# YuHang-max/3DSAD-main

Hardware: AMD Instinct MI355X
Metric: scenes/sec (16384-pt KITTI-shaped) through SA+cluster path (higher is better)
Workload: dtype f32

## Files before the change

3dsad-main_amd/csrc/ball_query.hip:

```cpp
#include "common.h"

namespace {

struct BQParams {
    float radii[SAD_MAX_RADII];
    int nsample[SAD_MAX_RADII];
    int32_t *idx[SAD_MAX_RADII];
    int32_t *cnt[SAD_MAX_RADII];
};

constexpr int BQ_WAVES = 4;

template <int NR, int CW>
__global__ __launch_bounds__(BQ_WAVES * 64) void ball_query_kernel(
    const float *__restrict__ xyz, const float *__restrict__ new_xyz,
    const float *__restrict__ radius_pc, BQParams prm, int N, int M) {
    const int lane = threadIdx.x & 63;
    const int wave = __builtin_amdgcn_readfirstlane(threadIdx.x >> 6);
    const int b = blockIdx.y;
    const int m0 = (blockIdx.x * BQ_WAVES + wave) * CW;
    const float *p = xyz + (size_t)b * N * 3;

    float cx[CW], cy[CW], cz[CW], r2[CW][NR];
    int cnt[CW][NR], first[CW][NR];
    bool active[CW];
    int ndone = 0;
#pragma unroll
    for (int c = 0; c < CW; ++c) {
        active[c] = (m0 + c) < M;
        const int m = active[c] ? m0 + c : M - 1;
        const float *q = new_xyz + ((size_t)b * M + m) * 3;
        cx[c] = q[0];
        cy[c] = q[1];
        cz[c] = q[2];
#pragma unroll
        for (int r = 0; r < NR; ++r) {
            float rad = prm.radii[r];
            if (radius_pc) rad = rad * radius_pc[(size_t)b * M + m];
            r2[c][r] = rad * rad;
            first[c][r] = 0;
            cnt[c][r] = active[c] ? 0 : prm.nsample[r];
            if (!active[c]) ++ndone;
        }
    }

    for (int base = 0; base < N && ndone < CW * NR; base += 64) {
        const int j = base + lane;
        const bool valid = j < N;
        const int jj = valid ? j : N - 1;
        const float px = p[jj * 3 + 0], py = p[jj * 3 + 1], pz = p[jj * 3 + 2];
#pragma unroll
        for (int c = 0; c < CW; ++c) {
            const float d = sad::d2f(px, py, pz, cx[c], cy[c], cz[c]);
#pragma unroll
            for (int r = 0; r < NR; ++r) {
                const bool in = valid && (d < r2[c][r]);
                const unsigned long long mask = __ballot(in);
                if (mask != 0ull && cnt[c][r] < prm.nsample[r]) {
                    const int slot = cnt[c][r] + __builtin_amdgcn_mbcnt_hi((unsigned)(mask >> 32), __builtin_amdgcn_mbcnt_lo((unsigned)mask, 0u));
                    if (in && slot < prm.nsample[r])
                        prm.idx[r][((size_t)b * M + (m0 + c)) * prm.nsample[r] + slot] = j;
                    if (cnt[c][r] == 0) first[c][r] = base + __builtin_ctzll(mask);
                    cnt[c][r] += __builtin_popcountll(mask);
                    if (cnt[c][r] >= prm.nsample[r]) ++ndone;
                }
            }
        }
    }
#pragma unroll
    for (int c = 0; c < CW; ++c) {
        if (!active[c]) continue;
#pragma unroll
        for (int r = 0; r < NR; ++r) {
            const int S = prm.nsample[r];
            const int n = cnt[c][r] < S ? cnt[c][r] : S;
            for (int s = n + lane; s < S; s += 64)
                prm.idx[r][((size_t)b * M + (m0 + c)) * S + s] = first[c][r];
            if (prm.cnt[r] && lane == 0) prm.cnt[r][(size_t)b * M + (m0 + c)] = n;
        }
    }
}

template <int NR>
void launch_bq(const float *xyz, const float *new_xyz, const float *radius_pc, const BQParams &prm,
               int B, int N, int M, hipStream_t st) {
    constexpr int CW = 4;
    dim3 grid((M + BQ_WAVES * CW - 1) / (BQ_WAVES * CW), B);
    hipLaunchKernelGGL((ball_query_kernel<NR, CW>), grid, dim3(BQ_WAVES * 64), 0, st, xyz, new_xyz,
                       radius_pc, prm, N, M);
}

__global__ __launch_bounds__(256) void knn_kernel(const float *__restrict__ xyz,
                                                  const float *__restrict__ new_xyz, int N, int M,
                                                  int K, int32_t *__restrict__ idx) {
    const int lane = threadIdx.x & 63;
    const int wave = __builtin_amdgcn_readfirstlane(threadIdx.x >> 6);
    const int b = blockIdx.y;
    const int m = blockIdx.x * 4 + wave;
    if (m >= M) return;
    const float *p = xyz + (size_t)b * N * 3;
    const float *q = new_xyz + ((size_t)b * M + m) * 3;
    const float cx = q[0], cy = q[1], cz = q[2];
    float ld = __builtin_inff();
    int lj = 0;
    float worst = __builtin_inff();
    int filled = 0;
    for (int base = 0; base < N; base += 64) {
        const int j = base + lane;
        const bool valid = j < N;
        const int jj = valid ? j : N - 1;
        const float d = sad::d2f(p[jj * 3 + 0], p[jj * 3 + 1], p[jj * 3 + 2], cx, cy, cz);
        unsigned long long mask = __ballot(valid && (d < worst || filled < K));
        while (mask) {
            const int l = __builtin_ctzll(mask);
            mask &= mask - 1;
            const float xd = __builtin_bit_cast(float, __builtin_amdgcn_readlane(__builtin_bit_cast(int, d), l));
            if (!(xd < worst) && filled >= K) continue;
            const int pos = __builtin_popcountll(__ballot(lane < filled && ld <= xd));
            const float ud = __shfl_up(ld, 1, 64);
            const int uj = __shfl_up(lj, 1, 64);
            if (lane > pos) {
                ld = ud;
                lj = uj;
            } else if (lane == pos) {
                ld = xd;
                lj = base + l;
            }
            if (lane >= K) ld = __builtin_inff();
            filled = filled < K ? filled + 1 : K;
            worst = filled < K ? __builtin_inff() : __builtin_bit_cast(float, __builtin_amdgcn_readlane(__builtin_bit_cast(int, ld), K - 1));
        }
    }
    if (lane < K) idx[((size_t)b * M + m) * K + lane] = lj;
}

int check_common(const char *fn, const void *xyz, const void *new_xyz, int B, int N, int M) {
    if (!xyz || !new_xyz) return sad::fail(SAD_EINVAL, "%s: NULL pointer", fn);
    if (B < 1 || N < 1 || M < 1) return sad::fail(SAD_EINVAL, "%s: need B,N,M >= 1 (B=%d N=%d M=%d)", fn, B, N, M);
    if (B > 65535) return sad::fail(SAD_EUNSUPPORTED, "%s: B=%d > 65535", fn, B);
    if ((size_t)N * 3 >= (1u << 31)) return sad::fail(SAD_EUNSUPPORTED, "%s: N too large", fn);
    return SAD_OK;
}

}

SAD_API int sad_ball_query_multi_f32(const float *xyz, const float *new_xyz, int n_radii,
                                     const float *radii, const float *radius_pc,
                                     const int *nsamples, int32_t *const *idx, int32_t *const *cnt,
                                     int B, int N, int M, sad_stream_t stream) {
    if (int e = check_common("sad_ball_query_multi_f32", xyz, new_xyz, B, N, M)) return e;
    SAD_REQUIRE(n_radii >= 1 && n_radii <= SAD_MAX_RADII, "sad_ball_query_multi_f32: n_radii=%d not in 1..%d", n_radii, SAD_MAX_RADII);
    SAD_REQUIRE(radii && nsamples && idx, "sad_ball_query_multi_f32: NULL parameter array");
    BQParams prm{};
    for (int r = 0; r < n_radii; ++r) {
        SAD_REQUIRE(nsamples[r] >= 1 && nsamples[r] <= 64, "sad_ball_query: nsample=%d not in 1..64", nsamples[r]);
        SAD_REQUIRE(idx[r], "sad_ball_query: NULL idx output");
        prm.radii[r] = radii[r];
        prm.nsample[r] = nsamples[r];
        prm.idx[r] = idx[r];
        prm.cnt[r] = cnt ? cnt[r] : nullptr;
    }
    hipStream_t st = (hipStream_t)stream;
    switch (n_radii) {
        case 1: launch_bq<1>(xyz, new_xyz, radius_pc, prm, B, N, M, st); break;
        case 2: launch_bq<2>(xyz, new_xyz, radius_pc, prm, B, N, M, st); break;
        case 3: launch_bq<3>(xyz, new_xyz, radius_pc, prm, B, N, M, st); break;
        default: launch_bq<4>(xyz, new_xyz, radius_pc, prm, B, N, M, st); break;
    }
    return sad::check_launch("sad_ball_query");
}

SAD_API int sad_ball_query_f32(const float *xyz, const float *new_xyz, float radius,
                               const float *radius_pc, int B, int N, int M, int S, int32_t *idx,
                               sad_stream_t stream) {
    const float radii[1] = {radius_pc ? 1.0f : radius};
    const int ns[1] = {S};
    int32_t *const outs[1] = {idx};
    return sad_ball_query_multi_f32(xyz, new_xyz, 1, radii, radius_pc, ns, outs, nullptr, B, N, M, stream);
}

SAD_API int sad_knn_f32(const float *xyz, const float *new_xyz, int B, int N, int M, int K,
                        int32_t *idx, sad_stream_t stream) {
    if (int e = check_common("sad_knn_f32", xyz, new_xyz, B, N, M)) return e;
    SAD_REQUIRE(idx, "sad_knn_f32: NULL idx");
    SAD_REQUIRE(K >= 1 && K <= 64 && K <= N, "sad_knn_f32: need 1 <= K <= min(64, N) (K=%d N=%d)", K, N);
    dim3 grid((M + 3) / 4, B);
    hipLaunchKernelGGL(knn_kernel, grid, dim3(256), 0, (hipStream_t)stream, xyz, new_xyz, N, M, K, idx);
    return sad::check_launch("sad_knn_f32");
}
```

Measured before the change: 8401.

## Stage small point clouds in registers and skip empty radius checks in ball query

For N up to 2048, each lane preloads all its point coordinates into registers up front, in NCH chunks, with an asm barrier to force the loads to issue early. The centroid width drops to 2 waves' worth on these paths. A per-centroid max-radius ballot lets a chunk skip all radius tests when no lane is inside, and also skips centroids whose radii are all full. Out-of-range lanes get NaN coordinates so the valid predicate can be dropped from the ballot. The aim is to cut global-load latency and redundant ballots, at the cost of higher register pressure and more template instantiations.

```diff
diff --git a/3dsad-main_amd/csrc/ball_query.hip b/3dsad-main_amd/csrc/ball_query.hip
--- a/3dsad-main_amd/csrc/ball_query.hip
+++ b/3dsad-main_amd/csrc/ball_query.hip
@@ -10,8 +10,13 @@
 };
 
 constexpr int BQ_WAVES = 4;
-
-template <int NR, int CW>
+constexpr int BQ_STAGED_MAX_N = 2048;
+
+__device__ __forceinline__ unsigned long long lanes_below(float a, float b) {
+    return __builtin_amdgcn_fcmpf(a, b, 4 );
+}
+
+template <int NR, int CW, int NCH>
 __global__ __launch_bounds__(BQ_WAVES * 64) void ball_query_kernel(
     const float *__restrict__ xyz, const float *__restrict__ new_xyz,
     const float *__restrict__ radius_pc, BQParams prm, int N, int M) {
@@ -21,10 +26,18 @@
     const int m0 = (blockIdx.x * BQ_WAVES + wave) * CW;
     const float *p = xyz + (size_t)b * N * 3;
 
-    float cx[CW], cy[CW], cz[CW], r2[CW][NR];
+    float cx[CW], cy[CW], cz[CW], r2[CW][NR], rmax2[CW];
     int cnt[CW][NR], first[CW][NR];
+    int nopen[CW];
     bool active[CW];
     int ndone = 0;
+    float pc[CW];
+#pragma unroll
+    for (int c = 0; c < CW; ++c) pc[c] = 1.0f;
+    if (radius_pc) {
+#pragma unroll
+        for (int c = 0; c < CW; ++c) pc[c] = radius_pc[(size_t)b * M + ((m0 + c) < M ? m0 + c : M - 1)];
+    }
 #pragma unroll
     for (int c = 0; c < CW; ++c) {
         active[c] = (m0 + c) < M;
@@ -33,38 +46,65 @@
         cx[c] = q[0];
         cy[c] = q[1];
         cz[c] = q[2];
+        nopen[c] = active[c] ? NR : 0;
 #pragma unroll
         for (int r = 0; r < NR; ++r) {
-            float rad = prm.radii[r];
-            if (radius_pc) rad = rad * radius_pc[(size_t)b * M + m];
+            const float rad = prm.radii[r] * pc[c];
             r2[c][r] = rad * rad;
+            rmax2[c] = r == 0 ? r2[c][0] : fmaxf(rmax2[c], r2[c][r]);
             first[c][r] = 0;
             cnt[c][r] = active[c] ? 0 : prm.nsample[r];
             if (!active[c]) ++ndone;
         }
     }
 
-    for (int base = 0; base < N && ndone < CW * NR; base += 64) {
+    auto chunk = [&](int base, float px, float py, float pz) {
         const int j = base + lane;
-        const bool valid = j < N;
-        const int jj = valid ? j : N - 1;
-        const float px = p[jj * 3 + 0], py = p[jj * 3 + 1], pz = p[jj * 3 + 2];
 #pragma unroll
         for (int c = 0; c < CW; ++c) {
             const float d = sad::d2f(px, py, pz, cx[c], cy[c], cz[c]);
+            if (nopen[c] == 0 || lanes_below(d, rmax2[c]) == 0ull) continue;
 #pragma unroll
             for (int r = 0; r < NR; ++r) {
-                const bool in = valid && (d < r2[c][r]);
-                const unsigned long long mask = __ballot(in);
+                const bool in = d < r2[c][r];
+                const unsigned long long mask = lanes_below(d, r2[c][r]);
                 if (mask != 0ull && cnt[c][r] < prm.nsample[r]) {
                     const int slot = cnt[c][r] + __builtin_amdgcn_mbcnt_hi((unsigned)(mask >> 32), __builtin_amdgcn_mbcnt_lo((unsigned)mask, 0u));
                     if (in && slot < prm.nsample[r])
                         prm.idx[r][((size_t)b * M + (m0 + c)) * prm.nsample[r] + slot] = j;
                     if (cnt[c][r] == 0) first[c][r] = base + __builtin_ctzll(mask);
                     cnt[c][r] += __builtin_popcountll(mask);
-                    if (cnt[c][r] >= prm.nsample[r]) ++ndone;
+                    if (cnt[c][r] >= prm.nsample[r]) {
+                        ++ndone;
+                        --nopen[c];
+                    }
                 }
             }
+        }
+    };
+
+    if constexpr (NCH > 0) {
+        float px[NCH], py[NCH], pz[NCH];
+#pragma unroll
+        for (int ch = 0; ch < NCH; ++ch) {
+            const int j = ch * 64 + lane;
+            const int jj = j < N ? j : N - 1;
+            px[ch] = p[jj * 3 + 0];
+            py[ch] = p[jj * 3 + 1];
+            pz[ch] = p[jj * 3 + 2];
+        }
+#pragma unroll
+        for (int ch = 0; ch < NCH; ++ch) asm volatile("" : "+v"(px[ch]), "+v"(py[ch]), "+v"(pz[ch]));
+#pragma unroll
+        for (int ch = 0; ch < NCH; ++ch) {
+            if (ch * 64 >= N || ndone >= CW * NR) break;
+            chunk(ch * 64, ch * 64 + lane < N ? px[ch] : __builtin_nanf(""), py[ch], pz[ch]);
+        }
+    } else {
+        for (int base = 0; base < N && ndone < CW * NR; base += 64) {
+            const int j = base + lane;
+            const int jj = j < N ? j : N - 1;
+            chunk(base, j < N ? p[jj * 3 + 0] : __builtin_nanf(""), p[jj * 3 + 1], p[jj * 3 + 2]);
         }
     }
 #pragma unroll
@@ -81,13 +121,24 @@
     }
 }
 
+template <int NR, int CW, int NCH>
+void launch_bq_as(const float *xyz, const float *new_xyz, const float *radius_pc, const BQParams &prm,
+                  int B, int N, int M, hipStream_t st) {
+    dim3 grid((M + BQ_WAVES * CW - 1) / (BQ_WAVES * CW), B);
+    hipLaunchKernelGGL((ball_query_kernel<NR, CW, NCH>), grid, dim3(BQ_WAVES * 64), 0, st, xyz, new_xyz,
+                       radius_pc, prm, N, M);
+}
+
 template <int NR>
 void launch_bq(const float *xyz, const float *new_xyz, const float *radius_pc, const BQParams &prm,
                int B, int N, int M, hipStream_t st) {
-    constexpr int CW = 4;
-    dim3 grid((M + BQ_WAVES * CW - 1) / (BQ_WAVES * CW), B);
-    hipLaunchKernelGGL((ball_query_kernel<NR, CW>), grid, dim3(BQ_WAVES * 64), 0, st, xyz, new_xyz,
-                       radius_pc, prm, N, M);
+    constexpr int CW = 2;
+    if (N <= 2 * 64) launch_bq_as<NR, CW, 2>(xyz, new_xyz, radius_pc, prm, B, N, M, st);
+    else if (N <= 4 * 64) launch_bq_as<NR, CW, 4>(xyz, new_xyz, radius_pc, prm, B, N, M, st);
+    else if (N <= 8 * 64) launch_bq_as<NR, CW, 8>(xyz, new_xyz, radius_pc, prm, B, N, M, st);
+    else if (N <= 16 * 64) launch_bq_as<NR, CW, 16>(xyz, new_xyz, radius_pc, prm, B, N, M, st);
+    else if (N <= BQ_STAGED_MAX_N) launch_bq_as<NR, CW, 32>(xyz, new_xyz, radius_pc, prm, B, N, M, st);
+    else launch_bq_as<NR, 4, 0>(xyz, new_xyz, radius_pc, prm, B, N, M, st);
 }
 
 __global__ __launch_bounds__(256) void knn_kernel(const float *__restrict__ xyz,
```

After: 8536, median of 6. 1.6% higher.
